# chacorp/latent-nerf-test

Measured on AMD Instinct MI355X. Metric: latent-frames/sec (64x64x4, 128^3 grid), render forward+backward, higher is better.
Workload: dtype bf16

## Files before the change

### latent-nerf-test_amd/csrc/grid_gather.hip

```cpp
#include "grid_shared.h"

namespace lnerf {

template <typename TT> struct CellRaw;
template <> struct CellRaw<uint16_t> {
    uint32_t d[8];
    __device__ __forceinline__ void load_pair(const uint16_t *lt, uint32_t row, int c) {
        const uint2 v = *reinterpret_cast<const uint2 *>(lt + (int64_t)row * 2);
        d[c] = v.x; d[c + 1] = v.y;
    }
    __device__ __forceinline__ void load_one(const uint16_t *lt, uint32_t row, int c) {
        d[c] = reinterpret_cast<const uint32_t *>(lt)[row];
    }
    __device__ __forceinline__ void load_quad(const uint16_t *lt, uint32_t r0, uint32_t r1, int c) {
        const uint4 v = *reinterpret_cast<const uint4 *>(lt + (int64_t)(r0 & ~3u) * 2);
        const uint32_t k0 = r0 & 3u, k1 = r1 & 3u;
        d[c] = (k0 & 2u) ? ((k0 & 1u) ? v.w : v.z) : ((k0 & 1u) ? v.y : v.x);
        d[c + 1] = (k1 & 2u) ? ((k1 & 1u) ? v.w : v.z) : ((k1 & 1u) ? v.y : v.x);
    }
    static constexpr bool kHasQuad = true;
    __device__ __forceinline__ void swap_pair(int c) { const uint32_t t = d[c]; d[c] = d[c + 1]; d[c + 1] = t; }
    __device__ __forceinline__ void zero() {
#pragma unroll
        for (int i = 0; i < 8; ++i) d[i] = 0u;
    }
    __device__ __forceinline__ void take_from_lane(int src) {
#pragma unroll
        for (int i = 0; i < 8; ++i) d[i] = (uint32_t)__builtin_amdgcn_ds_bpermute(src << 2, (int)d[i]);
    }
    __device__ __forceinline__ float2 get(int c) const {
        return make_float2(__uint_as_float(d[c] << 16), __uint_as_float(d[c] & 0xFFFF0000u));
    }
};
template <> struct CellRaw<float> {
    float2 d[8];
    __device__ __forceinline__ void load_pair(const float *lt, uint32_t row, int c) {
        const float4 v = *reinterpret_cast<const float4 *>(lt + (int64_t)row * 2);
        d[c] = make_float2(v.x, v.y); d[c + 1] = make_float2(v.z, v.w);
    }
    __device__ __forceinline__ void load_one(const float *lt, uint32_t row, int c) {
        d[c] = reinterpret_cast<const float2 *>(lt)[row];
    }
    __device__ __forceinline__ void load_quad(const float *, uint32_t, uint32_t, int) {}
    static constexpr bool kHasQuad = false;
    __device__ __forceinline__ void swap_pair(int c) { const float2 t = d[c]; d[c] = d[c + 1]; d[c + 1] = t; }
    __device__ __forceinline__ void zero() {
#pragma unroll
        for (int i = 0; i < 8; ++i) d[i] = make_float2(0.f, 0.f);
    }
    __device__ __forceinline__ void take_from_lane(int src) {
#pragma unroll
        for (int i = 0; i < 8; ++i) {
            d[i].x = __int_as_float(__builtin_amdgcn_ds_bpermute(src << 2, __float_as_int(d[i].x)));
            d[i].y = __int_as_float(__builtin_amdgcn_ds_bpermute(src << 2, __float_as_int(d[i].y)));
        }
    }
    __device__ __forceinline__ float2 get(int c) const { return d[c]; }
};

template <typename TT, typename TO>
__global__ void __launch_bounds__(256)
k_grid_forward(const float *__restrict__ xyzs, float bound, const TT *__restrict__ table, GridMeta meta, int64_t m_host,
               const int32_t *__restrict__ m_dev, int64_t level_stride, TO *__restrict__ feat, int pair_loads,
               int dedup_max_res) {
    int64_t M = m_host;
    if (m_dev) { const int64_t md = *m_dev; M = md < M ? md : M; }
    const TileMap tm = tile_map(0, meta.num_levels);
    const int l = tm.level;
    const float scale = meta.scales[l];
    const uint32_t res = (uint32_t)meta.res[l];
    const uint32_t off = (uint32_t)meta.offsets[l];
    const uint32_t hsize = (uint32_t)(meta.offsets[l + 1] - meta.offsets[l]);
    const TT *lt = table + (int64_t)off * 2;
    const bool dense = (uint64_t)(res + 1) * (res + 1) * (res + 1) <= (uint64_t)hsize;
    const bool pow2 = (hsize & (hsize - 1u)) == 0u;
    const bool dedup = (int)res <= dedup_max_res;
    const int lane = lane_id();
    for (int64_t tile = tm.tile0; tile * 256 < M; tile += tm.tstep) {
        const int64_t m = tile * 256 + threadIdx.x;
        const bool valid = m < M;
        LevelPos p;
        p.gx = p.gy = p.gz = 0u; p.fx = p.fy = p.fz = 0.f;
        if (valid) p = level_pos(xyzs, m, bound, scale);
        uint32_t rows[8];
        corner_rows(p.gx, p.gy, p.gz, res, hsize, rows, meta.blocked);
        bool fetch = valid;
        int src = lane;
        if (dedup) {
            const RunInfo ri = wave_cell_runs(p.gx, p.gy, p.gz, valid, lane);
            src = ri.start;
            fetch = valid && ri.start == lane;
        }
        CellRaw<TT> cell;
        cell.zero();
        if (fetch) {
            if (pair_loads && dense) {
#pragma unroll
                for (int c = 0; c < 8; c += 2) cell.load_pair(lt, rows[c], c);
            } else if (meta.blocked == 2) {
#pragma unroll
                for (int c = 0; c < 8; ++c) cell.load_one(lt, rows[c], c);
            } else if (pair_loads == 2 && CellRaw<TT>::kHasQuad && pow2 && (p.gx & 3u) != 3u) {
#pragma unroll
                for (int c = 0; c < 8; c += 2) cell.load_quad(lt, rows[c], rows[c + 1], c);
            } else if (pair_loads && pow2 && !(p.gx & 1u)) {
#pragma unroll
                for (int c = 0; c < 8; c += 2) {
                    cell.load_pair(lt, rows[c] & ~1u, c);
                    if (rows[c] & 1u) cell.swap_pair(c);
                }
            } else {
#pragma unroll
                for (int c = 0; c < 8; ++c) cell.load_one(lt, rows[c], c);
            }
        }
        if (dedup) cell.take_from_lane(src);
        float a0 = 0.f, a1 = 0.f;
#pragma unroll
        for (int c = 0; c < 8; ++c) {
            const uint32_t bx = c & 1, by = (c >> 1) & 1, bz = (c >> 2) & 1;
            const float wx = bx ? p.fx : 1.0f - p.fx;
            const float wy = by ? p.fy : 1.0f - p.fy;
            const float wz = bz ? p.fz : 1.0f - p.fz;
            const float w = (wx * wy) * wz;
            const float2 v = cell.get(c);
            a0 = fmaf(w, v.x, a0);
            a1 = fmaf(w, v.y, a1);
        }
        if (valid) Feat2<TO>::store(feat, (int64_t)l * level_stride + m, a0, a1);
    }
}

template <typename TG>
__global__ void __launch_bounds__(256)
k_grid_backward_atomic(const float *__restrict__ xyzs, float bound, const TG *__restrict__ dfeat, GridMeta meta,
                       int64_t m_host, const int32_t *__restrict__ m_dev, int64_t level_stride,
                       float *__restrict__ dtable, int variant) {
    int64_t M = m_host;
    if (m_dev) { const int64_t md = *m_dev; M = md < M ? md : M; }
    const TileMap tm = tile_map(variant, meta.num_levels);
    if (!tm.ok) return;
    const int l = tm.level;
    const float scale = meta.scales[l];
    const uint32_t res = (uint32_t)meta.res[l];
    const uint32_t off = (uint32_t)meta.offsets[l];
    const uint32_t hsize = (uint32_t)(meta.offsets[l + 1] - meta.offsets[l]);
    float *lt = dtable + (int64_t)off * 2;
    for (int64_t tile = tm.tile0; tile * 256 < M; tile += tm.tstep) {
        const int64_t m = tile * 256 + threadIdx.x;
        if (m >= M) continue;
        const LevelPos p = level_pos(xyzs, m, bound, scale);
        const float2 gg = Feat2<TG>::load(dfeat + ((int64_t)l * level_stride + m) * 2, 0);
        uint32_t rows[8];
        corner_rows(p.gx, p.gy, p.gz, res, hsize, rows, meta.blocked);
#pragma unroll
        for (int c = 0; c < 8; ++c) {
            const uint32_t bx = c & 1, by = (c >> 1) & 1, bz = (c >> 2) & 1;
            const uint32_t row = rows[c];
            const float wx = bx ? p.fx : 1.0f - p.fx;
            const float wy = by ? p.fy : 1.0f - p.fy;
            const float wz = bz ? p.fz : 1.0f - p.fz;
            const float w = (wx * wy) * wz;
            atomicAdd(lt + (int64_t)row * 2, w * gg.x);
            atomicAdd(lt + (int64_t)row * 2 + 1, w * gg.y);
        }
    }
}

static void launch_dims(int variant, int L, int64_t m_host, dim3 &grid) {
    const int64_t tiles = div_up(m_host, 256);
    if (variant == 0) {
        int64_t gx = tiles < 1 ? 1 : tiles;
        if (gx > 2048) gx = 2048;
        grid = dim3((unsigned)gx, (unsigned)L, 1);
    } else {
        const int lv_per_xcd = (L + 7) / 8;
        int64_t per_level = tiles < 1 ? 1 : tiles;
        if (per_level > 256) per_level = 256;
        grid = dim3((unsigned)(8 * lv_per_xcd * per_level), 1, 1);
    }
}

void launch_grid_backward_atomic(const float *xyzs, float bound, const float *dfeat, const GridMeta &meta, int64_t m_host,
                                 const int32_t *m_dev, int64_t level_stride, float *dtable, int variant, hipStream_t s) {
    dim3 grid;
    launch_dims(variant, meta.num_levels, m_host, grid);
    hipLaunchKernelGGL((k_grid_backward_atomic<float>), grid, dim3(256), 0, s, xyzs, bound, dfeat, meta, m_host, m_dev,
                       level_stride, dtable, variant);
}

}

using namespace lnerf;

extern "C" {

int lnerf_grid_encode_forward(const float *xyzs, float bound, const void *table, int table_dtype, int num_levels,
                              int level_dim, const int32_t *offsets_host, const float *scales_host,
                              const int32_t *res_host, int64_t m_host, const int32_t *m_dev, int64_t level_stride,
                              void *feat, int feat_dtype, int variant, lnerf_stream_t stream) {
    GridMeta meta;
    const int blocked = variant & (LNERF_GRID_BLOCKED | LNERF_GRID_TILED);
    variant &= ~(LNERF_GRID_BLOCKED | LNERF_GRID_TILED);
    int rc = fill_meta("grid_encode_forward", meta, num_levels, level_dim, offsets_host, scales_host, res_host, blocked);
    if (rc) return rc;
    LNERF_REQUIRE(m_host >= 0 && level_stride >= m_host, "grid_encode_forward: need 0 <= m_host <= level_stride");
    LNERF_REQUIRE(bound > 0.f, "grid_encode_forward: bound must be > 0");
    LNERF_REQUIRE(variant == 0, "grid_encode_forward: unknown variant %d", variant);
    LNERF_REQUIRE((table_dtype == LNERF_F32 || table_dtype == LNERF_BF16) &&
                      (feat_dtype == LNERF_F32 || feat_dtype == LNERF_BF16),
                  "grid_encode_forward: bad dtype tag");
    if (m_host == 0) return LNERF_OK;
    LNERF_REQUIRE(xyzs && table && feat, "grid_encode_forward: null pointer");
    dim3 grid;
    launch_dims(0, num_levels, m_host, grid);
    hipStream_t s = as_stream(stream);
#define LAUNCH_FWD(TT, TO)                                                                                         \
    hipLaunchKernelGGL((k_grid_forward<TT, TO>), grid, dim3(256), (size_t)g_gather_lds_pad, s, xyzs, bound, (const TT *)table, meta, m_host, \
                       m_dev, level_stride, (TO *)feat, g_gather_pairs, g_gather_dedup_res)
    if (table_dtype == LNERF_F32 && feat_dtype == LNERF_F32) LAUNCH_FWD(float, float);
    else if (table_dtype == LNERF_F32) LAUNCH_FWD(float, uint16_t);
    else if (feat_dtype == LNERF_F32) LAUNCH_FWD(uint16_t, float);
    else LAUNCH_FWD(uint16_t, uint16_t);
#undef LAUNCH_FWD
    LNERF_CHECK_LAUNCH("grid_encode_forward");
    return LNERF_OK;
}

}
```

Before: 2693.

## Micro-optimize grid forward gather addressing, index math and load paths

Rewrites the forward grid gather kernel to use 32-bit sample indices and byte offsets with scalar/vector register hints, so address arithmetic is cheaper. It also multiplies by a reciprocal when 2*bound is a power of two, and drops zero-initialisation of cells that are not fetched. Paired loads are enabled for blocked layouts, and bf16 stores use a native vector convert. The price is new host checks that cap sample counts and level sizes, plus reliance on inline-asm register constraints.

```diff
diff --git a/latent-nerf-test_amd/csrc/grid_gather.hip b/latent-nerf-test_amd/csrc/grid_gather.hip
--- a/latent-nerf-test_amd/csrc/grid_gather.hip
+++ b/latent-nerf-test_amd/csrc/grid_gather.hip
@@ -1,32 +1,39 @@
 #include "grid_shared.h"
 
 namespace lnerf {
+
+typedef uint32_t u32x2 __attribute__((ext_vector_type(2)));
+typedef float f32x4 __attribute__((ext_vector_type(4)));
+typedef u32x2 u32x2_dw __attribute__((aligned(4)));
+typedef f32x4 f32x4_dw __attribute__((aligned(4)));
+template <typename T> __device__ __forceinline__ T load_at(const char *base, uint32_t byte_off) {
+    return *reinterpret_cast<const T *>(base + byte_off);
+}
 
 template <typename TT> struct CellRaw;
 template <> struct CellRaw<uint16_t> {
     uint32_t d[8];
-    __device__ __forceinline__ void load_pair(const uint16_t *lt, uint32_t row, int c) {
-        const uint2 v = *reinterpret_cast<const uint2 *>(lt + (int64_t)row * 2);
+    __device__ __forceinline__ void load_pair(const char *lt, uint32_t row, int c) {
+        const u32x2 v = load_at<u32x2_dw>(lt, row << 2);
         d[c] = v.x; d[c + 1] = v.y;
     }
-    __device__ __forceinline__ void load_one(const uint16_t *lt, uint32_t row, int c) {
-        d[c] = reinterpret_cast<const uint32_t *>(lt)[row];
-    }
-    __device__ __forceinline__ void load_quad(const uint16_t *lt, uint32_t r0, uint32_t r1, int c) {
-        const uint4 v = *reinterpret_cast<const uint4 *>(lt + (int64_t)(r0 & ~3u) * 2);
+    __device__ __forceinline__ void load_one(const char *lt, uint32_t row, int c) { d[c] = load_at<uint32_t>(lt, row << 2); }
+    __device__ __forceinline__ void load_quad(const char *lt, uint32_t r0, uint32_t r1, int c) {
+        const uint4 v = load_at<uint4>(lt, (r0 & ~3u) << 2);
         const uint32_t k0 = r0 & 3u, k1 = r1 & 3u;
         d[c] = (k0 & 2u) ? ((k0 & 1u) ? v.w : v.z) : ((k0 & 1u) ? v.y : v.x);
         d[c + 1] = (k1 & 2u) ? ((k1 & 1u) ? v.w : v.z) : ((k1 & 1u) ? v.y : v.x);
     }
     static constexpr bool kHasQuad = true;
+    static constexpr uint32_t kMaxLevelRows = 1u << 30;
     __device__ __forceinline__ void swap_pair(int c) { const uint32_t t = d[c]; d[c] = d[c + 1]; d[c + 1] = t; }
-    __device__ __forceinline__ void zero() {
-#pragma unroll
-        for (int i = 0; i < 8; ++i) d[i] = 0u;
-    }
-    __device__ __forceinline__ void take_from_lane(int src) {
-#pragma unroll
-        for (int i = 0; i < 8; ++i) d[i] = (uint32_t)__builtin_amdgcn_ds_bpermute(src << 2, (int)d[i]);
+    __device__ __forceinline__ void unfetched() {
+#pragma unroll
+        for (int i = 0; i < 8; ++i) asm volatile("" : "=v"(d[i]));
+    }
+    __device__ __forceinline__ void take_from_lane(int src4) {
+#pragma unroll
+        for (int i = 0; i < 8; ++i) d[i] = (uint32_t)__builtin_amdgcn_ds_bpermute(src4, (int)d[i]);
     }
     __device__ __forceinline__ float2 get(int c) const {
         return make_float2(__uint_as_float(d[c] << 16), __uint_as_float(d[c] & 0xFFFF0000u));
@@ -34,76 +41,120 @@
 };
 template <> struct CellRaw<float> {
     float2 d[8];
-    __device__ __forceinline__ void load_pair(const float *lt, uint32_t row, int c) {
-        const float4 v = *reinterpret_cast<const float4 *>(lt + (int64_t)row * 2);
+    __device__ __forceinline__ void load_pair(const char *lt, uint32_t row, int c) {
+        const f32x4 v = load_at<f32x4_dw>(lt, row << 3);
         d[c] = make_float2(v.x, v.y); d[c + 1] = make_float2(v.z, v.w);
     }
-    __device__ __forceinline__ void load_one(const float *lt, uint32_t row, int c) {
-        d[c] = reinterpret_cast<const float2 *>(lt)[row];
-    }
-    __device__ __forceinline__ void load_quad(const float *, uint32_t, uint32_t, int) {}
+    __device__ __forceinline__ void load_one(const char *lt, uint32_t row, int c) { d[c] = load_at<float2>(lt, row << 3); }
+    __device__ __forceinline__ void load_quad(const char *, uint32_t, uint32_t, int) {}
     static constexpr bool kHasQuad = false;
+    static constexpr uint32_t kMaxLevelRows = 1u << 29;
     __device__ __forceinline__ void swap_pair(int c) { const float2 t = d[c]; d[c] = d[c + 1]; d[c + 1] = t; }
-    __device__ __forceinline__ void zero() {
-#pragma unroll
-        for (int i = 0; i < 8; ++i) d[i] = make_float2(0.f, 0.f);
-    }
-    __device__ __forceinline__ void take_from_lane(int src) {
+    __device__ __forceinline__ void unfetched() {
+#pragma unroll
+        for (int i = 0; i < 8; ++i) asm volatile("" : "=v"(d[i].x), "=v"(d[i].y));
+    }
+    __device__ __forceinline__ void take_from_lane(int src4) {
 #pragma unroll
         for (int i = 0; i < 8; ++i) {
-            d[i].x = __int_as_float(__builtin_amdgcn_ds_bpermute(src << 2, __float_as_int(d[i].x)));
-            d[i].y = __int_as_float(__builtin_amdgcn_ds_bpermute(src << 2, __float_as_int(d[i].y)));
+            d[i].x = __int_as_float(__builtin_amdgcn_ds_bpermute(src4, __float_as_int(d[i].x)));
+            d[i].y = __int_as_float(__builtin_amdgcn_ds_bpermute(src4, __float_as_int(d[i].y)));
         }
     }
     __device__ __forceinline__ float2 get(int c) const { return d[c]; }
 };
 
+__device__ __forceinline__ LevelPos gather_level_pos(float x, float y, float z, float bound, float inv_two_b, float scale) {
+    float px = x + bound, py = y + bound, pz = z + bound;
+    if (inv_two_b != 0.f) {
+        px = px * inv_two_b; py = py * inv_two_b; pz = pz * inv_two_b;
+    } else {
+        const float two_b = 2.0f * bound;
+        px = px / two_b; py = py / two_b; pz = pz / two_b;
+    }
+    px = px * scale; py = py * scale; pz = pz * scale;
+    px = px + 0.5f; py = py + 0.5f; pz = pz + 0.5f;
+    const float flx = floorf(px), fly = floorf(py), flz = floorf(pz);
+    LevelPos r;
+    r.gx = (uint32_t)(int)flx; r.gy = (uint32_t)(int)fly; r.gz = (uint32_t)(int)flz;
+    r.fx = px - flx; r.fy = py - fly; r.fz = pz - flz;
+    return r;
+}
+
+typedef float f32x2 __attribute__((ext_vector_type(2)));
+typedef __bf16 bf16x2 __attribute__((ext_vector_type(2)));
+__device__ __forceinline__ uint32_t bf16_pair(float a, float b) {
+    const f32x2 v = {a, b};
+    const bf16x2 h = __builtin_convertvector(v, bf16x2);
+    uint32_t r;
+    __builtin_memcpy(&r, &h, sizeof(r));
+    return r;
+}
+template <typename TO> __device__ __forceinline__ void store_feat(char *fb, uint32_t lane_in_tile, float a, float b);
+template <> __device__ __forceinline__ void store_feat<float>(char *fb, uint32_t lane_in_tile, float a, float b) {
+    *reinterpret_cast<float2 *>(fb + lane_in_tile * 8u) = make_float2(a, b);
+}
+template <> __device__ __forceinline__ void store_feat<uint16_t>(char *fb, uint32_t lane_in_tile, float a, float b) {
+    *reinterpret_cast<uint32_t *>(fb + lane_in_tile * 4u) = bf16_pair(a, b);
+}
+
 template <typename TT, typename TO>
 __global__ void __launch_bounds__(256)
-k_grid_forward(const float *__restrict__ xyzs, float bound, const TT *__restrict__ table, GridMeta meta, int64_t m_host,
-               const int32_t *__restrict__ m_dev, int64_t level_stride, TO *__restrict__ feat, int pair_loads,
-               int dedup_max_res) {
-    int64_t M = m_host;
-    if (m_dev) { const int64_t md = *m_dev; M = md < M ? md : M; }
+k_grid_forward(const float *__restrict__ xyzs, float bound, float inv_two_b, const TT *__restrict__ table, GridMeta meta,
+               uint32_t m_host, const int32_t *__restrict__ m_dev, int64_t level_stride, TO *__restrict__ feat,
+               int pair_loads, int dedup_max_res) {
+    uint32_t M = m_host;
+    if (m_dev) { const int32_t md = *m_dev; M = md < 0 ? 0u : ((uint32_t)md < M ? (uint32_t)md : M); }
     const TileMap tm = tile_map(0, meta.num_levels);
     const int l = tm.level;
     const float scale = meta.scales[l];
     const uint32_t res = (uint32_t)meta.res[l];
     const uint32_t off = (uint32_t)meta.offsets[l];
-    const uint32_t hsize = (uint32_t)(meta.offsets[l + 1] - meta.offsets[l]);
-    const TT *lt = table + (int64_t)off * 2;
-    const bool dense = (uint64_t)(res + 1) * (res + 1) * (res + 1) <= (uint64_t)hsize;
-    const bool pow2 = (hsize & (hsize - 1u)) == 0u;
+    const char *lt = reinterpret_cast<const char *>(table + (int64_t)off * 2);
     const bool dedup = (int)res <= dedup_max_res;
     const int lane = lane_id();
-    for (int64_t tile = tm.tile0; tile * 256 < M; tile += tm.tstep) {
-        const int64_t m = tile * 256 + threadIdx.x;
-        const bool valid = m < M;
+    const uint32_t tid = threadIdx.x;
+    for (uint32_t tile = (uint32_t)tm.tile0; tile * 256u < M; tile += (uint32_t)tm.tstep) {
+        const bool valid = tile * 256u + tid < M;
+        uint32_t hsize = (uint32_t)(meta.offsets[l + 1] - meta.offsets[l]);
+        asm volatile("" : "+s"(hsize));
+        const bool dense = (uint64_t)(res + 1) * (res + 1) * (res + 1) <= (uint64_t)hsize;
+        const bool pow2 = (hsize & (hsize - 1u)) == 0u;
+        const bool blocked = meta.blocked == 1 && !dense;
         LevelPos p;
-        p.gx = p.gy = p.gz = 0u; p.fx = p.fy = p.fz = 0.f;
-        if (valid) p = level_pos(xyzs, m, bound, scale);
+        if (valid) {
+            uint64_t tile_off = (uint64_t)tile * (256u * 12u);
+            uint32_t poff = tid * 12u;
+            asm volatile("" : "+s"(tile_off), "+v"(poff));
+            const char *pb = reinterpret_cast<const char *>(xyzs) + tile_off;
+            const float *pp = reinterpret_cast<const float *>(pb + poff);
+            p = gather_level_pos(pp[0], pp[1], pp[2], bound, inv_two_b, scale);
+        } else {
+            asm volatile("" : "=v"(p.gx), "=v"(p.gy), "=v"(p.gz), "=v"(p.fx), "=v"(p.fy), "=v"(p.fz));
+        }
         uint32_t rows[8];
         corner_rows(p.gx, p.gy, p.gz, res, hsize, rows, meta.blocked);
         bool fetch = valid;
-        int src = lane;
+        int src4;
         if (dedup) {
             const RunInfo ri = wave_cell_runs(p.gx, p.gy, p.gz, valid, lane);
-            src = ri.start;
+            src4 = ri.start << 2;
             fetch = valid && ri.start == lane;
+        } else {
+            asm volatile("" : "=v"(src4));
         }
         CellRaw<TT> cell;
-        cell.zero();
         if (fetch) {
-            if (pair_loads && dense) {
+            const bool x_in_group = (p.gx & 3u) != 3u;
+            const bool hashed = pair_loads && meta.blocked == 0 && pow2 && !dense;
+            const bool quads = hashed && pair_loads == 2 && CellRaw<TT>::kHasQuad && x_in_group;
+            if (pair_loads && (dense || (blocked && x_in_group))) {
 #pragma unroll
                 for (int c = 0; c < 8; c += 2) cell.load_pair(lt, rows[c], c);
-            } else if (meta.blocked == 2) {
-#pragma unroll
-                for (int c = 0; c < 8; ++c) cell.load_one(lt, rows[c], c);
-            } else if (pair_loads == 2 && CellRaw<TT>::kHasQuad && pow2 && (p.gx & 3u) != 3u) {
+            } else if (quads) {
 #pragma unroll
                 for (int c = 0; c < 8; c += 2) cell.load_quad(lt, rows[c], rows[c + 1], c);
-            } else if (pair_loads && pow2 && !(p.gx & 1u)) {
+            } else if (hashed && !(p.gx & 1u)) {
 #pragma unroll
                 for (int c = 0; c < 8; c += 2) {
                     cell.load_pair(lt, rows[c] & ~1u, c);
@@ -113,8 +164,10 @@
 #pragma unroll
                 for (int c = 0; c < 8; ++c) cell.load_one(lt, rows[c], c);
             }
-        }
-        if (dedup) cell.take_from_lane(src);
+        } else {
+            cell.unfetched();
+        }
+        if (dedup) cell.take_from_lane(src4);
         float a0 = 0.f, a1 = 0.f;
 #pragma unroll
         for (int c = 0; c < 8; ++c) {
@@ -127,7 +180,13 @@
             a0 = fmaf(w, v.x, a0);
             a1 = fmaf(w, v.y, a1);
         }
-        if (valid) Feat2<TO>::store(feat, (int64_t)l * level_stride + m, a0, a1);
+        if (valid) {
+            uint64_t tile_off = ((uint64_t)l * (uint64_t)level_stride + (uint64_t)tile * 256u) * (2 * sizeof(TO));
+            uint32_t lane_in_tile = tid;
+            asm volatile("" : "+s"(tile_off), "+v"(lane_in_tile));
+            char *fb = reinterpret_cast<char *>(feat) + tile_off;
+            store_feat<TO>(fb, lane_in_tile, a0, a1);
+        }
     }
 }
 
@@ -212,12 +271,21 @@
                   "grid_encode_forward: bad dtype tag");
     if (m_host == 0) return LNERF_OK;
     LNERF_REQUIRE(xyzs && table && feat, "grid_encode_forward: null pointer");
+    LNERF_REQUIRE(m_host <= (int64_t)INT32_MAX, "grid_encode_forward: m_host must be < 2^31 (32-bit sample indices)");
+    const uint32_t max_rows = table_dtype == LNERF_F32 ? CellRaw<float>::kMaxLevelRows : CellRaw<uint16_t>::kMaxLevelRows;
+    for (int l = 0; l < num_levels; ++l)
+        LNERF_REQUIRE((uint32_t)(offsets_host[l + 1] - offsets_host[l]) <= max_rows,
+                      "grid_encode_forward: level %d is larger than 4 GiB (32-bit byte offsets)", l);
+    const float two_b = 2.0f * bound;
+    uint32_t two_b_bits;
+    memcpy(&two_b_bits, &two_b, sizeof(two_b_bits));
+    const float inv_two_b = (two_b_bits & 0x007FFFFFu) == 0u ? 1.0f / two_b : 0.f;
     dim3 grid;
     launch_dims(0, num_levels, m_host, grid);
     hipStream_t s = as_stream(stream);
 #define LAUNCH_FWD(TT, TO)                                                                                         \
-    hipLaunchKernelGGL((k_grid_forward<TT, TO>), grid, dim3(256), (size_t)g_gather_lds_pad, s, xyzs, bound, (const TT *)table, meta, m_host, \
-                       m_dev, level_stride, (TO *)feat, g_gather_pairs, g_gather_dedup_res)
+    hipLaunchKernelGGL((k_grid_forward<TT, TO>), grid, dim3(256), (size_t)g_gather_lds_pad, s, xyzs, bound, inv_two_b, (const TT *)table, meta, \
+                       (uint32_t)m_host, m_dev, level_stride, (TO *)feat, g_gather_pairs, g_gather_dedup_res)
     if (table_dtype == LNERF_F32 && feat_dtype == LNERF_F32) LAUNCH_FWD(float, float);
     else if (table_dtype == LNERF_F32) LAUNCH_FWD(float, uint16_t);
     else if (feat_dtype == LNERF_F32) LAUNCH_FWD(uint16_t, float);
```

Measured after the change: 2727 (median of 6 runs). 1.3% higher.
